# bayesml/BayesML

Measured on AMD Instinct MI355X. Metric: GMM-VB E+M samples/sec at K=64,D=128,N=1e7; 1/2/4/8-GPU scaling, higher is better.
Workload: dtype f64; 1 GPU; GMM-VB K=64 D=128 N=10000000 rows/GPU x 1 GPU, x stored f32, one VB iteration per step (c3 of BASELINE.json configs); classes=64, degree=128, rows_per_gpu=10000000, rows_total=10000000, x_storage=f32, parallelism=rows1, row_tiles=1

## Files before the change

### bayesml_amd/csrc/capi_estep.hip

```cpp
#include "capi_internal.h"

namespace {

struct Pass {
    gmmvb_workspace* ws;
    const void* x_dev;
    int64_t ldx, n_rows;
    hipStream_t st;
    int is64;
    bool vec;
    int sel_grid;
    double pairs;
    EstepArgs a{};
    EstepI8Args a8{};
    RecArrays rec{};
    bool i8 = false;
    bool prunable = false;
    bool prev_lists = false, can_project = false, own_known = false, tmeta_was_valid = false;
    bool quiet_was_valid = false;
    int mode = kPassDense;
    bool settle = false, proof_capable = false;
    double skip_margin = -1.0;
    bool counted = false, proof_ran = false, tmeta_kept = false, projected = false, filtered = false, emission_to_hmm = false,
         sorted_now = false;
// ... 116 lines not shown
                       estep_gather_rows_per_wg(ws->T, is64), ws->plan);
    hipError_t e = hipGetLastError();
    span_end(ws, st);
    if (e != hipSuccess) return e;
    span_begin(ws, kSpanGather, st);
    e = launch_estep_gather_dev(ws->T, is64, vec, 2 * ws->num_cu, st, a, ws->lists, ws->npad, ws->counts, ws->plan, thr,
                                thr ? ws->exit_ctr : nullptr, 0.0f);
    span_end(ws, st);
    ++ws->passes[7];
    return e;
}

}

extern "C" {


bool cal_wanted(gmmvb_workspace* ws, int what, double pairs) {
    return ws->opt_calibrate && ws->cal_ev[0] != nullptr && !((ws->pt.measured >> what) & 1) && ws->cal_pairs[what] == 0.0 &&
           pairs >= (double)(int64_t(1) << 23) && ws->hmm == nullptr;
}
void cal_mark(gmmvb_workspace* ws, int what, double pairs, hipStream_t st) {
    note_hip(ws, hipEventRecord(ws->cal_ev[2 * what + 1], st));
    ws->cal_pairs[what] = pairs;
}
void cal_poll(gmmvb_workspace* ws) {
    for (int what = 0; what < 3; ++what) {
        if (ws->cal_pairs[what] <= 0.0 || hipEventQuery(ws->cal_ev[2 * what + 1]) != hipSuccess) continue;
        float ms = 0.0f;
        if (hipEventElapsedTime(&ms, ws->cal_ev[2 * what], ws->cal_ev[2 * what + 1]) == hipSuccess) {
            double ns = (double)ms * 1e6 / ws->cal_pairs[what];
            if (what == 2) ns += 0.010 * tri_pairs(ws->T) / 36.0;
            const bool took = ws->pt.take(what, ns);
            if (ws->opt_debug)
                std::fprintf(stderr, "[gmmvb] policy table: %s %.4f ns per pair %s (prune below %.3f, dense again above %.3f, list M below %.3f)\n",
                             what == 0 ? "dense E" : (what == 1 ? "dense M" : "bound pass"), ns, took ? "taken" : "out of range: literal kept",
                             ws->pt.prune_below(), ws->pt.dense_again_above(), ws->pt.list_m_below());
            if (!took) ws->pt.measured |= 8 << what;
            ws->cal_pairs[what] = (took || ++ws->cal_tries[what] >= 3) ? -1.0 : 0.0;
        } else {
            ws->cal_pairs[what] = -1.0;
        }
    }
}

}

namespace {

hipError_t proof_round(gmmvb_workspace* ws, hipStream_t st, const int* blk_base, int sel_grid, int64_t n_rows, float* ub) {
    if (ws->opt_proof_blocked && ws->slabs &&
        estep_i8_proof_work_bytes(ws->K, n_rows) <= ws->scratch->bytes[kBuf_slabs])
        return launch_estep_i8_proof_blocked(ws->D, ws->num_cu, st, ws->xq, ws->xqe, ws->img_i8b, ws->cvec, ws->K, ws->lists,
                                             ws->npad, ws->counts, blk_base, sel_grid, ws->slabs, ub, ws->lnrho, ws->npad);
    hipLaunchKernelGGL(gather_plan_kernel, dim3(1), dim3(64), 0, st, ws->counts, ws->K, estep_i8_pairs_per_chunk(), ws->plan);
    return launch_estep_i8_proof(ws->D, ws->num_cu, st, ws->xq, ws->xqe, ws->img_i8b, ws->cvec, ws->K, ws->lists, ws->npad,
                                 ws->counts, ws->plan, ub, ws->lnrho, ws->npad);
}

int Pass::run_generic() {
    const int R = generic_rows(ws->D);
    const dim3 g((unsigned)((n_rows + R - 1) / R), (unsigned)ws->K);
    const size_t lds = (size_t)ws->D * R * sizeof(double);
    span_begin(ws, kSpanEstepMain, st);
    if (is64)
        hipLaunchKernelGGL(estep_generic_kernel<double>, g, dim3(64), lds, st, (const double*)x_dev, ldx, n_rows, ws->D,
                           ws->gen_u, ws->gen_m, ws->cvec, R, ws->lnrho, ws->npad);
    else
        hipLaunchKernelGGL(estep_generic_kernel<float>, g, dim3(64), lds, st, (const float*)x_dev, ldx, n_rows, ws->D,
                           ws->gen_u, ws->gen_m, ws->cvec, R, ws->lnrho, ws->npad);
    span_end(ws, st);
    if (phase_events(ws)) {
        note_hip(ws, hipEventRecord(ws->ev[1], st));
        ws->ev_e = true;
    }
    phase_closed = true;
    span_begin(ws, kSpanLse, st);
    hipLaunchKernelGGL(row_lse_kernel, dim3((unsigned)((n_rows + kLseRows - 1) / kLseRows)), dim3(256), 0, st, ws->lnrho,
                       ws->npad, n_rows, ws->K, ws->lse, nullptr, nullptr, 1);
    span_end(ws, st);
    hipError_t eg = hipGetLastError();
    if (eg != hipSuccess) return fail(GMMVB_EHIP, "estep_generic launch", eg);
    ++ws->passes[0];
    ws->rec_live = ws->rec_valid = false;
    ws->evaluated = pairs;
    std::snprintf(ws->info, sizeof(ws->info), "estep_generic_f64<D=%d> grid=%ux%ux64 rows/workgroup=%d", ws->D, g.x, g.y, R);
    name = nullptr;
    return GMMVB_OK;
}

int Pass::run_dense() {
    const bool valu16 = ws->estep_variant == kEstepValu16 && ws->tri != nullptr;
    emission_to_hmm = ws->T == 1 && !ws->wide && !i8 && !ws->sorted && hmm_fused_emission(ws->hmm);
    rpw = ws->wide ? estep_rows_rows_per_wg()
                     : (i8 ? estep_i8_rows_per_wg() : (valu16 ? estep_rows16_rows_per_wg() : estep_rows_per_wg(ws->estep_variant, ws->T, is64)));
    grid = (n_rows + rpw - 1) / rpw;
    if (grid > (1 << 20)) grid = 1 << 20;
    span_begin(ws, kSpanEstepMain, st);
    const bool cal_e = !ws->wide && !i8 && !emission_to_hmm && !valu16 && cal_wanted(ws, 0, pairs);
    if (cal_e) note_hip(ws, hipEventRecord(ws->cal_ev[0], st));
    hipError_t e = ws->wide ? launch_estep_rows(ws->T, is64, (int)grid, st, a, &name)
                            : (i8 ? launch_estep_i8(is64, vec, (int)grid, st, a8, &name)
                                  : (emission_to_hmm ? hmm_launch_emission16(ws->hmm, is64, vec, st, a, &name)
                                     : (valu16 ? launch_estep_rows16(is64, vec, (int)grid, st, a, ws->tri, &name)
                                            : launch_estep(ws->estep_variant, ws->T, is64, vec, (int)grid, st, a, &name))));
    if (cal_e) cal_mark(ws, 0, pairs, st);
    span_end(ws, st);
// ... 415 lines not shown
```

### bayesml_amd/csrc/estep_i8.h

```cpp
#pragma once
#include "common.h"

#include <type_traits>

namespace gmmvb {

typedef int i4v __attribute__((ext_vector_type(4)));
typedef int i16v __attribute__((ext_vector_type(16)));

constexpr int kDigits = 6;
constexpr int kBoundDigits = 3;

__host__ __device__ constexpr int i8_blocks(int D) { return (D + 31) / 32; }
__host__ __device__ constexpr int i8_img_bytes(int nd, int t32) {
    return (tri_pairs(t32) * nd * 1024 + (nd == kBoundDigits ? t32 * 128 + 32 : t32 * 512) + 1023) / 1024 * 1024;
}
__host__ __device__ constexpr int i8_kb(int nd, int t32) {
    const int kb = (64 * 1024) / i8_img_bytes(nd, t32);
    return kb < 1 ? 1 : (kb > 8 ? 8 : kb);
}
__host__ __device__ constexpr double i8_err(int nd, int t32) {
    double w = 1.0;
    for (int i = 0; i < 7 * nd; ++i) w *= 0.5;
    return w * (2.0 + 1.02 * (nd - 1)) * 32.0 * t32 * 1.000001;
}

template <int ND>
__device__ __forceinline__ void digits_of(double t, int (&d)[ND]) {
#pragma unroll
    for (int a = 0; a < ND; ++a) {
        const double r = __builtin_rint(t);
        d[a] = (int)r;
        t = (t - r) * 128.0;
    }
}

template <int ND>
__device__ __forceinline__ void pack_i8_image(const double* us, int ld, const double* dm, int D, int T32, int img_bytes,
                                              unsigned char* __restrict__ im, double* row_scale ,
                                              double* row_max, double* row_beta, int* row_bad) {
    const int P = tri_pairs(T32);
    double* consts = reinterpret_cast<double*>(im + P * ND * 1024);
    for (int j = threadIdx.x; j < 32 * T32; j += blockDim.x) {
        double mx = 0.0, bias = 0.0, abias = 0.0;
        bool bad = false;
        if (j < D) {
            for (int i = 0; i <= j; ++i) {
                const double v = us[j * ld + i];
                bad |= !(fabs(v) <= 1.7976931348623157e308);
                mx = fmax(mx, fabs(v));
                bias = fma(v, dm[i], bias);
                abias = fma(fabs(v), fabs(dm[i]), abias);
            }
        }
// ... 518 lines not shown
            const int64_t e = chunk0 + ((int64_t)t * NW + wave) * 32 + c;
            return list[e < count ? e : count - 1];
        };
        auto request = [&](int idx, i4v (&xd)[ND][T32], int64_t& row, int& en) {
            row = idx;
            const unsigned char* src = xq + row * RS + 16 * h;
#pragma unroll
            for (int a = 0; a < ND; ++a)
#pragma unroll
                for (int it = 0; it < T32; ++it) xd[a][it] = *reinterpret_cast<const i4v*>(src + a * 32 * T32 + 32 * it);
            en = xqe[row];
        };
        auto evaluate = [&](int t, const i4v (&xd)[ND][T32], int64_t row, int en) {
            const bool ok = en != kNoDigits;
            i8_lane_consts lc;
            lc.c[0] = lc.c[1] = lc.c[2] = 0.0;
            lc.c2f = ok ? (float)ldexp(1.0, en - 12 - 7 * (ND - 1)) : 0.0f;
            lc.cef = ok ? (float)(ldexp(1.0, en) * i8_err(ND, T32) * 1.0001) : __builtin_huge_valf();
            float q_lo, q_hi;
            if (T32 > 1 && wave >= NW / 2)
                estep_i8_two_sided<T32, true>(im_lds, xd, lc, lane, h, q_lo, q_hi);
            else
                estep_i8_two_sided<T32, false>(im_lds, xd, lc, lane, h, q_lo, q_hi);
            const int64_t e = chunk0 + ((int64_t)t * NW + wave) * 32 + c;
            if (h == 0 && e < count) {
                const double up = fma(-0.5 * (double)q_lo, 1.0 - 1.52587890625e-05, ck + 1e-12 * fabs(ck));
                const double lo = fma(-0.5 * (double)q_hi, 1.0 + 1.52587890625e-05, ck - 1e-12 * fabs(ck));
                if (ub) ub[(int64_t)k * npad + row] = __double2float_ru(up);
                lb[(int64_t)k * npad + row] = (lo == lo) ? lo : -__builtin_huge_val();
            }
        };
        i4v xa[ND][T32], xb[ND][T32];
        int64_t ra = 0, rb = 0;
        int ea = 0, eb = 0;
        int i1 = nt > 1 ? entry(1) : 0;
        if (nt > 0) request(entry(0), xa, ra, ea);
        for (int t = 0; t < nt; t += 2) {
            const int i2 = t + 2 < nt ? entry(t + 2) : 0;
            if (t + 1 < nt) request(i1, xb, rb, eb);
            evaluate(t, xa, ra, ea);
            if (t + 1 >= nt) break;
            const int i3 = t + 3 < nt ? entry(t + 3) : 0;
            if (t + 2 < nt) request(i2, xa, ra, ea);
            evaluate(t + 1, xb, rb, eb);
            i1 = i3;
        }
    }
}


constexpr int kProofSuperRows = 4096;
constexpr int kProofItem = 256;
constexpr int kProofXcds = 8;

__device__ __forceinline__ void proof_unit(const int* __restrict__ blk_base, const int* __restrict__ counts, int nblk, int s,
                                           int k, int K, int& lo, int& hi) {
    constexpr int BS = kProofSuperRows / 256;
    const int b0 = s * BS, b1 = b0 + BS;
    lo = blk_base[(int64_t)b0 * K + k];
    hi = b1 < nblk ? blk_base[(int64_t)b1 * K + k] : counts[k];
}

__global__ __launch_bounds__(256) void proof_units_kernel(const int* __restrict__ blk_base ,
                                                          const int* __restrict__ counts, int K, int nblk,
                                                          int* __restrict__ cum , int* __restrict__ tot) {
    __shared__ int sc[256];
    const int s = blockIdx.x, k = threadIdx.x;
    int n = 0;
    if (k < K) {
        int lo, hi;
        proof_unit(blk_base, counts, nblk, s, k, K, lo, hi);
        n = (hi - lo + kProofItem - 1) / kProofItem;
    }
    sc[k] = n;
    __syncthreads();
    for (int o = 1; o < 256; o <<= 1) {
        const int v = k >= o ? sc[k - o] : 0;
        __syncthreads();
        sc[k] += v;
        __syncthreads();
    }
    if (k < K) cum[(int64_t)s * (K + 1) + k] = sc[k] - n;
    if (k == 255) {
        cum[(int64_t)s * (K + 1) + K] = sc[255];
        tot[s] = sc[255];
    }
}

__global__ __launch_bounds__(1024) void proof_order_kernel(const int* __restrict__ tot, int n_super, int* __restrict__ xb,
                                                           int* __restrict__ xtot) {
    __shared__ int sc[1024];
    const int x = blockIdx.x, t = threadIdx.x;
    const int nx = n_super > x ? (n_super - x + kProofXcds - 1) / kProofXcds : 0;
    const int per = (nx + 1023) / 1024;
    const int j0 = t * per, j1 = j0 + per < nx ? j0 + per : nx;
    int sum = 0;
    for (int j = j0; j < j1; ++j) sum += tot[x + kProofXcds * j];
    sc[t] = sum;
    __syncthreads();
    for (int o = 1; o < 1024; o <<= 1) {
        const int v = t >= o ? sc[t - o] : 0;
        __syncthreads();
        sc[t] += v;
        __syncthreads();
    }
    int run = sc[t] - sum;
    for (int j = j0; j < j1; ++j) {
        xb[x + kProofXcds * j] = run;
        run += tot[x + kProofXcds * j];
    }
    if (t == 1023) xtot[x] = sc[1023];
}

__global__ __launch_bounds__(256) void proof_items_kernel(const int* __restrict__ blk_base, const int* __restrict__ counts, int K,
                                                          int nblk, const int* __restrict__ cum, const int* __restrict__ xb,
                                                          const int* __restrict__ xtot, i4v* __restrict__ items) {
    const int s = blockIdx.x, k = threadIdx.x;
    if (k >= K) return;
    int first = 0;
    for (int q = 0; q < s % kProofXcds; ++q) first += xtot[q];
    int lo, hi;
    proof_unit(blk_base, counts, nblk, s, k, K, lo, hi);
    i4v* dst = items + first + xb[s] + cum[(int64_t)s * (K + 1) + k];
    for (int e = lo; e < hi; e += kProofItem) *dst++ = i4v{k, e, hi - e < kProofItem ? hi - e : kProofItem, s};
}

template <int T32>
__global__ __launch_bounds__(512) void estep_i8_proof_blocked(const unsigned char* __restrict__ xq, const signed char* __restrict__ xqe,
                                                              const unsigned char* __restrict__ img ,
                                                              const double* __restrict__ cvec, int K,
                                                              const int* __restrict__ lists , int64_t cap,
                                                              const i4v* __restrict__ items, const int* __restrict__ xtot,
                                                              float* __restrict__ ub , double* __restrict__ lb ,
                                                              int64_t npad) {
    constexpr int ND = kBoundDigits, NW = 8;
    constexpr int IMGB = i8_img_bytes(ND, T32);
    constexpr int64_t RS = i8_digit_row_bytes(T32);
    constexpr int NS = T32 <= 3 ? 3 : 2;
    constexpr int NI = (IMGB + 512 * 16 - 1) / (512 * 16);
    __shared__ __attribute__((aligned(16))) unsigned char smem[2][IMGB];
    const int tid = threadIdx.x;
    const int lane = tid & 63;
    const int wave = __builtin_amdgcn_readfirstlane(tid >> 6);
    const int c = lane & 31, h = lane >> 5;
    const int x = (int)(blockIdx.x % kProofXcds), j = (int)(blockIdx.x / kProofXcds), W = (int)(gridDim.x / kProofXcds);
    int first = 0;
    for (int q = 0; q < x; ++q) first += xtot[q];
    const int n_items = xtot[x];
    const i4v* my = items + first;
    if (n_items <= j) return;
    auto desc = [&](int t) -> i4v {
        const int i = j + t * W;
        i4v d = my[i < n_items ? i : n_items - 1];
        if (i >= n_items) d[3] = -1;
        return d;
    };
    auto entry = [&](const i4v& d) -> int {
        const int o = wave * 32 + c;
        return lists[(int64_t)d[0] * cap + d[1] + (o < d[2] ? o : d[2] - 1)];
    };
    auto image_load = [&](int k, i4v (&ir)[NI]) {
        const unsigned char* src = img + (int64_t)k * IMGB;
#pragma unroll
        for (int q = 0; q < NI; ++q) {
            const int o = (q * 512 + tid) * 16;
            ir[q] = *reinterpret_cast<const i4v*>(src + (o < IMGB ? o : IMGB - 16));
        }
    };
    auto image_store = [&](int buf, const i4v (&ir)[NI]) {
#pragma unroll
        for (int q = 0; q < NI; ++q)
            if ((q * 512 + tid) * 16 < IMGB) *reinterpret_cast<i4v*>(&smem[buf][(q * 512 + tid) * 16]) = ir[q];
    };
    auto request = [&](int idx, i4v (&xd)[ND][T32], int64_t& row, int& en) {
        row = idx;
        const unsigned char* src = xq + row * RS + 16 * h;
#pragma unroll
        for (int a = 0; a < ND; ++a)
#pragma unroll
            for (int it = 0; it < T32; ++it) xd[a][it] = *reinterpret_cast<const i4v*>(src + a * 32 * T32 + 32 * it);
        en = xqe[row];
    };
    auto evaluate = [&](const i4v& d, int buf, const i4v (&xd)[ND][T32], int64_t row, int en) {
        if (d[3] < 0 || wave * 32 >= d[2]) return;
        const unsigned im_lds = (unsigned)(uintptr_t)((__attribute__((address_space(3))) unsigned char*)smem[buf]);
        const bool ok = en != kNoDigits;
        i8_lane_consts lc;
        lc.c[0] = lc.c[1] = lc.c[2] = 0.0;
        lc.c2f = ok ? (float)ldexp(1.0, en - 12 - 7 * (ND - 1)) : 0.0f;
        lc.cef = ok ? (float)(ldexp(1.0, en) * i8_err(ND, T32) * 1.0001) : __builtin_huge_valf();
        float q_lo, q_hi;
        if (T32 > 1 && wave >= NW / 2)
            estep_i8_two_sided<T32, true>(im_lds, xd, lc, lane, h, q_lo, q_hi);
        else
            estep_i8_two_sided<T32, false>(im_lds, xd, lc, lane, h, q_lo, q_hi);
        if (h == 0 && wave * 32 + c < d[2]) {
            const int k = d[0];
            const double ck = cvec[k];
            const double up = fma(-0.5 * (double)q_lo, 1.0 - 1.52587890625e-05, ck + 1e-12 * fabs(ck));
            const double lo = fma(-0.5 * (double)q_hi, 1.0 + 1.52587890625e-05, ck - 1e-12 * fabs(ck));
            if (ub) ub[(int64_t)k * npad + row] = __double2float_ru(up);
            lb[(int64_t)k * npad + row] = (lo == lo) ? lo : -__builtin_huge_val();
        }
    };
    i4v xs[NS][ND][T32];
    int64_t rows[NS];
    int ens[NS];
    i4v dd[NS + 2];
#pragma unroll
    for (int i = 0; i < NS + 2; ++i) dd[i] = desc(i);
    i4v ir[NI];
    image_load(dd[0][0], ir);
#pragma unroll
    for (int q = 0; q < NS; ++q) {
        rows[q] = 0;
        ens[q] = 0;
        if (q + 1 < NS) request(entry(dd[q]), xs[q], rows[q], ens[q]);
    }
    int e_next = entry(dd[NS - 1]);
    constexpr int UNR = (T32 <= 2 ? 4 : 2) * NS;
    for (int t = 0; dd[0][3] >= 0; t += UNR) {
#pragma unroll
        for (int p = 0; p < UNR; ++p) {
            const int buf = (t + p) & 1;
            image_store(buf, ir);
            __syncthreads();
            image_load(dd[1][0], ir);
            const int e_new = entry(dd[NS]);
            request(e_next, xs[(p + NS - 1) % NS], rows[(p + NS - 1) % NS], ens[(p + NS - 1) % NS]);
            e_next = e_new;
            const i4v dn = desc(t + p + NS + 2);
            evaluate(dd[0], buf, xs[p % NS], rows[p % NS], ens[p % NS]);
#pragma unroll
            for (int i = 0; i < NS + 1; ++i) dd[i] = dd[i + 1];
            dd[NS + 1] = dn;
        }
    }
}

}
```

### bayesml_amd/csrc/estep_i8_inst.hip

```cpp
#include <cstdint>
#include <cstdlib>
#include <mutex>
#include "aux_kernels.h"
#include "estep_i8.h"
#include "launch.h"

namespace gmmvb {

int estep_i8_image_bytes(int D, int bound) { return i8_img_bytes(bound ? kBoundDigits : kDigits, i8_blocks(D)); }
int estep_i8_rows_per_wg() { return 8 * 32; }

constexpr int kPackThreads = 512;
__global__ __launch_bounds__(kPackThreads) void pack_images_kernel(const double* __restrict__ u, const double* __restrict__ m,
                                                                    const double* __restrict__ c_src, const double* __restrict__ pivot_src,
                                                                    int K, int D, int T, int img_len, double* __restrict__ img,
                                                                    double* __restrict__ c_dst, double* __restrict__ pivot_dst,
                                                                    int T32, unsigned char* __restrict__ img6, int img6_bytes,
                                                                    unsigned char* __restrict__ img3, int img3_bytes) {
    extern __shared__ double us[];
    __shared__ double row_scale[128], row_max[128], row_beta[128];
    __shared__ int row_bad[128];
    const int k = blockIdx.x, kind = blockIdx.y;
    const int ld = D | 1;
    double* mv = us + D * ld;
    const double* uk = u + (int64_t)k * D * D;
    for (int e = threadIdx.x; e < D * D; e += kPackThreads) {
        const int i = e / D, j = e - i * D;
        if (j <= i) us[i * ld + j] = uk[e];
    }
    for (int i = threadIdx.x; i < D; i += kPackThreads) {
        const double mi = m[(int64_t)k * D + i];
        mv[i] = kind == 0 ? mi : mi - pivot_src[i];
    }
    __syncthreads();
    if (kind == 0) {
        if (threadIdx.x == 0) c_dst[k] = c_src[k];
        if (pivot_dst && k == 0)
            for (int f = threadIdx.x; f < D; f += kPackThreads) pivot_dst[f] = pivot_src[f];
        pack_f64_image(us, ld, mv, D, T, img_len, img + (int64_t)k * img_len);
    } else if (kind == 1 && img6) {
        pack_i8_image<kDigits>(us, ld, mv, D, T32, img6_bytes, img6 + (int64_t)k * img6_bytes, row_scale, row_max, row_beta, row_bad);
    } else {
        pack_i8_image<kBoundDigits>(us, ld, mv, D, T32, img3_bytes, img3 + (int64_t)k * img3_bytes, row_scale, row_max, row_beta,
                                    row_bad);
    }
}

hipError_t launch_pack_images(const double* u, const double* m, const double* c_src, const double* pivot_src, int K, int D, int T,
                              int img_len, double* img, double* cvec, double* pivot_dst, unsigned char* img6, unsigned char* img3,
                              hipStream_t st) {
    if (D > 128 || ((img6 || img3) && !pivot_dst)) return hipErrorInvalidValue;
    static std::mutex mu;
    static bool asked[64] = {};
    int dev = 0;
    hipError_t e = hipGetDevice(&dev);
    if (e != hipSuccess) return e;
    {
        std::lock_guard<std::mutex> lock(mu);
// ... 51 lines not shown
    if (t32 < 1 || t32 > 4 || tb < 1 || tb > t32) return hipErrorInvalidValue;
    *name = names[t32][tb];
#define BC(T, B) \
    if (t32 == T && tb == B) return pick_x<kBoundDigits, true, T, B>(x_is_f64, vec, grid, st, a);
    BC(1, 1) BC(2, 1) BC(2, 2) BC(3, 1) BC(3, 2) BC(3, 3) BC(4, 1) BC(4, 2) BC(4, 3) BC(4, 4)
#undef BC
    return hipErrorInvalidValue;
}

int64_t estep_i8_digit_row_bytes(int D) { return i8_digit_row_bytes(i8_blocks(D)); }

hipError_t launch_x_digits(const void* x, int x_is_f64, int64_t ldx, int64_t n_rows, int D, const double* pivot,
                           unsigned char* xq, signed char* xqe, hipStream_t st) {
    const int t32 = i8_blocks(D);
    if (t32 < 1 || t32 > 4) return hipErrorInvalidValue;
    const unsigned grid = (unsigned)((n_rows + 31) / 32);
    if (x_is_f64)
        hipLaunchKernelGGL(x_digits_kernel<double>, dim3(grid), dim3(256), 0, st, static_cast<const double*>(x), ldx, n_rows, D,
                           t32, pivot, xq, xqe);
    else
        hipLaunchKernelGGL(x_digits_kernel<float>, dim3(grid), dim3(256), 0, st, static_cast<const float*>(x), ldx, n_rows, D,
                           t32, pivot, xq, xqe);
    return hipGetLastError();
}

int estep_i8_pairs_per_chunk() { return i8_pairs_per_chunk(); }

hipError_t launch_estep_i8_proof(int D, int grid, hipStream_t st, const unsigned char* xq, const signed char* xqe,
                                 const unsigned char* img, const double* cvec, int K, const int* lists, int64_t cap,
                                 const int* counts, const int* plan, float* ub, double* lb, int64_t npad) {
    if (K > 256) return hipErrorInvalidValue;
    grid *= 2;
#define PC(T)                                                                                                              \
    case T:                                                                                                                \
        hipLaunchKernelGGL((estep_i8_proof<T>), dim3(grid), dim3(512), 0, st, xq, xqe, img, cvec, K, lists, cap, counts,   \
                           plan, ub, lb, npad);                                                                            \
        return hipGetLastError();
    switch (i8_blocks(D)) {
        PC(1) PC(2) PC(3) PC(4)
    }
#undef PC
    return hipErrorInvalidValue;
}


int64_t estep_i8_proof_work_bytes(int K, int64_t n_rows) {
    const int64_t nblk = (n_rows + 255) / 256;
    const int64_t n_super = (nblk * 256 + kProofSuperRows - 1) / kProofSuperRows;
    const int64_t head = ((2 * n_super + kProofXcds + 3) / 4 * 4 + (n_super * (K + 1) + 3) / 4 * 4) * (int64_t)sizeof(int);
    const int64_t items = n_rows * (int64_t)K / kProofItem + n_super * K + 1;
    return head + items * (int64_t)sizeof(i4v);
}

hipError_t launch_estep_i8_proof_blocked(int D, int num_cu, hipStream_t st, const unsigned char* xq, const signed char* xqe,
                                         const unsigned char* img, const double* cvec, int K, const int* lists, int64_t cap,
                                         const int* counts, const int* blk_base, int nblk, void* work, float* ub, double* lb,
                                         int64_t npad) {
    if (K > 256 || nblk < 1 || !work || ((uintptr_t)work & 15)) return hipErrorInvalidValue;
    const int n_super = (int)(((int64_t)nblk * 256 + kProofSuperRows - 1) / kProofSuperRows);
    int* tot = static_cast<int*>(work);
    int* xb = tot + n_super;
    int* xtot = xb + n_super;
    int* cum = tot + (2 * (int64_t)n_super + kProofXcds + 3) / 4 * 4;
    i4v* items = reinterpret_cast<i4v*>(cum + ((int64_t)n_super * (K + 1) + 3) / 4 * 4);
    hipLaunchKernelGGL(proof_units_kernel, dim3(n_super), dim3(256), 0, st, blk_base, counts, K, nblk, cum, tot);
    hipLaunchKernelGGL(proof_order_kernel, dim3(kProofXcds), dim3(1024), 0, st, tot, n_super, xb, xtot);
    hipLaunchKernelGGL(proof_items_kernel, dim3(n_super), dim3(256), 0, st, blk_base, counts, K, nblk, cum, xb, xtot, items);
    const int per_cu = i8_blocks(D) == 1 ? 2 : 1;
    const int grid = kProofXcds * ((per_cu * num_cu + kProofXcds - 1) / kProofXcds);
#define PB(T)                                                                                                              \
    case T:                                                                                                                \
        hipLaunchKernelGGL((estep_i8_proof_blocked<T>), dim3(grid), dim3(512), 0, st, xq, xqe, img, cvec, K, lists, cap,   \
                           items, xtot, ub, lb, npad);                                                                     \
        return hipGetLastError();
    switch (i8_blocks(D)) {
        PB(1) PB(2) PB(3) PB(4)
    }
#undef PB
    return hipErrorInvalidValue;
}

}
```

### bayesml_amd/csrc/launch.h

```cpp
#pragma once
#include <hip/hip_runtime.h>
#include <stdint.h>

#include "workspace_plan.h"

struct gmmvb_hmm_state;

namespace gmmvb {

struct EstepArgs {
    const void* x; int64_t ldx; int64_t n_rows; int D;
    const double* img; const double* cvec; int K;
    double* lnrho; int64_t npad;
};
struct MstepArgs {
    const void* x; int64_t ldx; int64_t n_rows; int D;
    const double* pivot; const double* lnrho; const double* lse; const double* aux; int64_t npad;
    int K; int KG; int S; int64_t rows_per_split; int direct_r; double* slabs;
};

int estep_rows_per_wg(int variant, int T, int x_is_f64);
int estep_threads(int variant);
int estep_image_doubles(int T);
int estep_tri_image_doubles();
int estep_rows16_rows_per_wg();
hipError_t launch_pack_tri16(const double* u, const double* m, int K, int D, double* tri, hipStream_t st);
hipError_t launch_estep_rows16(int x_is_f64, bool vec, int grid, hipStream_t st, const EstepArgs& a, const double* tri,
                               const char** name);
hipError_t hmm_launch_emission16(::gmmvb_hmm_state* h, int x_is_f64, bool vec, hipStream_t st, const EstepArgs& a, const char** name);
int estep_bound_blocks(int T);
int estep_gather_rows_per_wg(int T, int x_is_f64);
hipError_t launch_estep_gather_dev(int T, int x_is_f64, bool vec, int grid, hipStream_t st, const EstepArgs& a,
                                   const int* lists, int64_t cap, const int* counts_dev, const int* plan_dev,
                                   const float* thr = nullptr ,
                                   unsigned long long* exits = nullptr ,
                                   float margin = 0.0f );
int64_t estep_i8_digit_row_bytes(int D);
hipError_t launch_x_digits(const void* x, int x_is_f64, int64_t ldx, int64_t n_rows, int D, const double* pivot,
                           unsigned char* xq, signed char* xqe, hipStream_t st);
int64_t proj_image_len(int K, int D);
int64_t proj_const_len(int K);
hipError_t launch_proj_table(const double* u, const double* m, const double* cvec, const double* pivot, int K, int D,
                             unsigned char* gimg, void* gconst, hipStream_t st);
hipError_t launch_proj_tile_ref(const int* counts, int K, int64_t n_tiles, int* tile_ref, hipStream_t st);
struct ProjectArgs {
    const unsigned char* xq; const signed char* xqe;
    const unsigned char* gimg; const void* gconst; const int* tile_ref;
    const double* lnrho; int64_t npad; int64_t n_rows; int K; int D; const double* drift; const double* cvec;
    unsigned short* rec_k; float* rec_d; float* rec_B; unsigned char* rec_exact; unsigned char* rec_sel; unsigned char* rec_flags;
    unsigned long long* masks; int* blk; double* epart; double* opart;
    unsigned char* lock; float* dlock; float* rthr; const unsigned char* lcomp;
    unsigned long long* pmask; int* pblk; int proof_all; int own_fresh; unsigned long long* cand_ctr;
};
hipError_t launch_rec_project(int grid, hipStream_t st, const ProjectArgs& a);
hipError_t launch_proj_filter(int grid, hipStream_t st, const ProjectArgs& a);
int estep_i8_pairs_per_chunk();
hipError_t launch_estep_i8_proof(int D, int grid, hipStream_t st, const unsigned char* xq, const signed char* xqe,
                                 const unsigned char* img, const double* cvec, int K, const int* lists, int64_t cap,
                                 const int* counts, const int* plan, float* ub, double* lb, int64_t npad);
int64_t estep_i8_proof_work_bytes(int K, int64_t n_rows);
hipError_t launch_estep_i8_proof_blocked(int D, int num_cu, hipStream_t st, const unsigned char* xq, const signed char* xqe,
                                         const unsigned char* img, const double* cvec, int K, const int* lists, int64_t cap,
                                         const int* counts, const int* blk_base, int nblk, void* work, float* ub, double* lb,
                                         int64_t npad);
struct EstepI8Args {
    const void* x; int64_t ldx; int64_t n_rows; int D;
    const unsigned char* img; const double* pivot; const double* cvec; int K;
    double* lnrho; int64_t npad;
    int* khat = nullptr;
    float* ub = nullptr;
};
int estep_i8_image_bytes(int D, int bound);
int estep_i8_rows_per_wg();
hipError_t launch_pack_images(const double* u, const double* m, const double* c_src, const double* pivot_src, int K, int D, int T,
                              int img_len, double* img, double* cvec, double* pivot_dst, unsigned char* img6, unsigned char* img3,
                              hipStream_t st);
hipError_t launch_estep_i8(int x_is_f64, bool vec, int grid, hipStream_t st, const EstepI8Args& a, const char** name);
hipError_t launch_estep_i8_bound(int x_is_f64, bool vec, int tb, int grid, hipStream_t st, const EstepI8Args& a,
                                 const char** name);
int mstep_components_per_wg(int T, bool pre);
int mstep_threads(int T, bool pre);
hipError_t launch_estep(int variant, int T, int x_is_f64, bool vec, int grid, hipStream_t st, const EstepArgs& a,
                        const char** name);
hipError_t launch_mstep(int T, int x_is_f64, bool vec, bool pre, int grid, hipStream_t st, const MstepArgs& a,
                        const char** name);

hipError_t launch_mstep_small(int grid, hipStream_t st, const MstepArgs& a, int KGW, int cw, const char** name);
hipError_t launch_mstep_wide(int T, int grid, hipStream_t st, const MstepArgs& a, const char** name);
hipError_t launch_estep_rows(int T, int x_is_f64, int grid, hipStream_t st, const EstepArgs& a, const char** name);
int estep_rows_rows_per_wg();
hipError_t launch_hmm_mstep_small(int grid, hipStream_t st, const MstepArgs& a, int KGW, const double* gamma_tm, int Kp,
                                  bool sparse, const char** name);

struct MstepListArgs {
    const double* xc; const double* lnrho; const double* lse;
    const int* lists; int64_t cap; const int* counts; int* plan; int cap_chunks; int r_min;
    int64_t npad; int K; double* slabs;
    const float* x32 = nullptr; int64_t ldx = 0; int64_t n_rows = 0; int D = 0; const double* pivot = nullptr;
    int direct_r = 0;
    int num_cu = 0;
    int runs_cap = 0;
};
hipError_t launch_mstep_list(int T, int grid, hipStream_t st, const MstepListArgs& a, const char** name, int* runs);

}
```

### bayesml_amd/csrc/workspace_plan.h

```cpp
#pragma once
#include <stdint.h>

#include <algorithm>
#include <cstdlib>
#include <cstring>
#include <type_traits>
#include <vector>

#include "../../include/gmmvb.h"

namespace gmmvb {

enum EstepVariant { kEstepLds = 0, kEstepDirect = 1, kEstepLds8 = 2, kEstepI8 = 3, kEstepValu16 = 4 };
inline int64_t round_up(int64_t v, int64_t m) { return (v + m - 1) / m * m; }

inline bool not_zero(const char* v) { return !(v && std::strcmp(v, "0") == 0); }
inline bool is(const char* v, const char* word) { return v && std::strcmp(v, word) == 0; }
template <typename Lookup>
inline const char* dev_switch(Lookup&& lookup, const char* name) {
    const char* on = lookup("GMMVB_DEBUG");
    return (on && on[0] != '\0' && on[0] != '0') ? lookup(name) : nullptr;
}

struct WorkspaceOptions {
    bool sparse = true;
    int prune = 1;
    int variant_asked = -1;
    bool sort_rows = true;
    double settle_margin = 1e300;
    bool opt_proof = true;
    bool opt_proof_all = true;
    bool opt_proof_blocked = true;
    bool opt_lazy = true;
    int opt_project = 0;
    bool opt_regroup_margin = true;
    bool gather_exit = true;
    bool cache_on = true;
    bool opt_carry_off = false;
    bool opt_hmm_mstep_dense = false;
    bool opt_calibrate = true;
    bool opt_quiet_tiles = true;
    bool opt_mlist_xc = false;
    int opt_mlist_runs = 0;
    int opt_sweep_run = 0;
    bool opt_debug = false;

    template <typename Lookup>
    static WorkspaceOptions read(Lookup&& lookup) {
        auto dev = [&lookup](const char* name) { return dev_switch(lookup, name); };
        WorkspaceOptions o;
        o.sparse = not_zero(lookup("GMMVB_MSTEP_SPARSE"));
        o.prune = is(lookup("GMMVB_ESTEP_PRUNE"), "0") ? 0 : (is(lookup("GMMVB_ESTEP_PRUNE"), "force") ? 2 : 1);
        const char* variant = dev("GMMVB_ESTEP_VARIANT");
        o.variant_asked = is(variant, "lds8") ? kEstepLds8 : is(variant, "direct") ? kEstepDirect : is(variant, "lds4") ? kEstepLds
                          : is(variant, "i8") ? kEstepI8 : -1;
        o.sort_rows = not_zero(dev("GMMVB_SORT_ROWS"));
        if (const char* v = dev("GMMVB_SETTLE_MARGIN")) o.settle_margin = std::atof(v);
        o.opt_proof = not_zero(dev("GMMVB_PROOF"));
        o.opt_proof_all = !is(dev("GMMVB_PROOF"), "settled");
        o.opt_proof_blocked = not_zero(dev("GMMVB_PROOF_BLOCKED"));
        o.opt_lazy = not_zero(dev("GMMVB_SWEEP_LAZY"));
        o.opt_project = is(dev("GMMVB_PROJECT"), "filter") ? 1 : (is(dev("GMMVB_PROJECT"), "only") ? 2 : 0);
        o.opt_regroup_margin = not_zero(dev("GMMVB_REGROUP_MARGIN"));
        o.gather_exit = not_zero(dev("GMMVB_GATHER_EXIT"));
        o.cache_on = not_zero(dev("GMMVB_MSTEP_CACHE"));
        o.opt_carry_off = dev("GMMVB_ESTEP_CARRY_OFF") != nullptr;
        o.opt_hmm_mstep_dense = dev("GMMVB_HMM_MSTEP_DENSE") != nullptr;
        o.opt_calibrate = not_zero(dev("GMMVB_POLICY_CALIBRATE"));
        o.opt_quiet_tiles = not_zero(dev("GMMVB_QUIET_TILES"));
        if (const char* v = dev("GMMVB_MLIST_XC")) o.opt_mlist_xc = v[0] == '1';
        if (const char* v = dev("GMMVB_MLIST_RUNS")) o.opt_mlist_runs = std::max(0, std::atoi(v));
        if (const char* v = dev("GMMVB_SWEEP_RUN")) o.opt_sweep_run = std::max(0, std::atoi(v));
        o.opt_debug = lookup("GMMVB_DEBUG") && lookup("GMMVB_DEBUG")[0] == '2';
        return o;
    }
};

constexpr int kSweepRunDefault = 2;
inline int sweep_run_length(int K, int asked) {
    if (K > 128) return 1;
    const int want = asked > 0 ? asked : kSweepRunDefault;
    return want >= 4 ? 4 : (want >= 2 ? 2 : 1);
}
template <typename F>
inline void dispatch_sweep_run(int run, F&& f) {
    if (run == 4) return f(std::integral_constant<int, 4>{});
    if (run == 2) return f(std::integral_constant<int, 2>{});
    return f(std::integral_constant<int, 1>{});
}

struct KernelSizes {
    int max_tiles = 0, t1_splits = 0, sel_rows = 0, lse_rows = 0, scan_parts = 0, rec_slots = 0;
    int mstep_components_per_wg = 0;
    int slab_len = 0, estep_image_doubles = 0, estep_tri_image_doubles = 0, estep_bound_blocks = 0;
    int estep_i8_image_bytes = 0, estep_i8_bound_image_bytes = 0;
    int64_t estep_i8_digit_row_bytes = 0, proj_image_len = 0, proj_const_len = 0;
    int generic_rows = 0;
};

inline bool wide_features(int D, int max_tiles) { return D > 16 * max_tiles && D <= 32 * max_tiles; }
inline int feature_tiles(int D, int max_tiles) {
    const int T = (D + 15) / 16;
    return wide_features(D, max_tiles) ? 2 * ((T + 1) / 2) : T;
}

struct WorkspaceShape : WorkspaceOptions {
    int K = 0, D = 0, x_dtype = 0, num_cu = 0, T = 0;
    int64_t max_rows = 0, npad = 0;
    bool wide = false;
    bool generic = false;
    int KG = 0, S_cap = 0, img_len = 0, estep_variant = 0, gen_S = 1, img_i8_len = 0, img_i8b_len = 0;
    int64_t split_rows = 0, xc_len = 0;
    bool has_lists = false;
};

inline WorkspaceShape make_shape(int K, int D, int x_dtype, int64_t max_rows, int num_cu, const WorkspaceOptions& opt,
                                 const KernelSizes& ks) {
    WorkspaceShape s;
    s.K = K;
    s.D = D;
    s.x_dtype = x_dtype;
    s.max_rows = max_rows;
    s.num_cu = num_cu;
    s.T = feature_tiles(D, ks.max_tiles);
    s.wide = wide_features(D, ks.max_tiles);
    s.generic = D > 32 * ks.max_tiles;
    s.npad = round_up(max_rows, 64);
    if (s.generic) {
        s.sparse = s.sort_rows = s.cache_on = false;
        s.prune = 0;
        s.gen_S = (int)std::min<int64_t>(64, std::max<int64_t>(1, max_rows / 16384));
        return s;
    }
    static_cast<WorkspaceOptions&>(s) = opt;
    s.KG = (K + ks.mstep_components_per_wg - 1) / ks.mstep_components_per_wg;
    s.S_cap = std::max(8, (int)round_up(((int64_t)(s.T == 1 ? ks.t1_splits : 4) * num_cu + s.KG - 1) / s.KG, 8));
    s.split_rows = round_up(std::max<int64_t>(64, (16 << 20) / (16 * s.T * 8)), 64);
    s.S_cap = (int)std::max<int64_t>(s.S_cap, round_up((max_rows + s.split_rows - 1) / s.split_rows, 8));
    s.img_len = ks.estep_image_doubles;
    s.estep_variant = s.T == 1 ? kEstepValu16 : kEstepLds8;
    if (!s.wide && opt.variant_asked >= 0) s.estep_variant = opt.variant_asked;
// ... 195 lines not shown
```

Measured before the change: 6.580 billion samples/s.

## Assign contiguous item stretches per workgroup in blocked proof and skip redundant image restaging

```diff
diff --git a/bayesml_amd/csrc/capi_estep.hip b/bayesml_amd/csrc/capi_estep.hip
--- a/bayesml_amd/csrc/capi_estep.hip
+++ b/bayesml_amd/csrc/capi_estep.hip
@@ -192,7 +192,8 @@
     if (ws->opt_proof_blocked && ws->slabs &&
         estep_i8_proof_work_bytes(ws->K, n_rows) <= ws->scratch->bytes[kBuf_slabs])
         return launch_estep_i8_proof_blocked(ws->D, ws->num_cu, st, ws->xq, ws->xqe, ws->img_i8b, ws->cvec, ws->K, ws->lists,
-                                             ws->npad, ws->counts, blk_base, sel_grid, ws->slabs, ub, ws->lnrho, ws->npad);
+                                             ws->npad, ws->counts, blk_base, sel_grid, ws->slabs, ws->opt_proof_run, ws->opt_debug,
+                                             ub, ws->lnrho, ws->npad);
     hipLaunchKernelGGL(gather_plan_kernel, dim3(1), dim3(64), 0, st, ws->counts, ws->K, estep_i8_pairs_per_chunk(), ws->plan);
     return launch_estep_i8_proof(ws->D, ws->num_cu, st, ws->xq, ws->xqe, ws->img_i8b, ws->cvec, ws->K, ws->lists, ws->npad,
                                  ws->counts, ws->plan, ub, ws->lnrho, ws->npad);
diff --git a/bayesml_amd/csrc/estep_i8.h b/bayesml_amd/csrc/estep_i8.h
--- a/bayesml_amd/csrc/estep_i8.h
+++ b/bayesml_amd/csrc/estep_i8.h
@@ -1,5 +1,6 @@
 #pragma once
 #include "common.h"
+#include "workspace_plan.h"
 
 #include <type_traits>
 
@@ -624,6 +625,7 @@
 constexpr int kProofSuperRows = 4096;
 constexpr int kProofItem = 256;
 constexpr int kProofXcds = 8;
+static_assert(kProofRunMax == kProofSuperRows / kProofItem, "a stretch holds at most the items of one full unit");
 
 __device__ __forceinline__ void proof_unit(const int* __restrict__ blk_base, const int* __restrict__ counts, int nblk, int s,
                                            int k, int K, int& lo, int& hi) {
@@ -703,6 +705,7 @@
                                                               const double* __restrict__ cvec, int K,
                                                               const int* __restrict__ lists , int64_t cap,
                                                               const i4v* __restrict__ items, const int* __restrict__ xtot,
+                                                              int run_asked ,
                                                               float* __restrict__ ub , double* __restrict__ lb ,
                                                               int64_t npad) {
     constexpr int ND = kBoundDigits, NW = 8;
@@ -720,9 +723,15 @@
     for (int q = 0; q < x; ++q) first += xtot[q];
     const int n_items = xtot[x];
     const i4v* my = items + first;
-    if (n_items <= j) return;
-    auto desc = [&](int t) -> i4v {
-        const int i = j + t * W;
+    const int G = proof_run_length(n_items, W, run_asked);
+    if (n_items <= j * G) return;
+    int nx_base = j * G, nx_off = 0;
+    auto next_desc = [&]() -> i4v {
+        const int i = nx_base + nx_off;
+        if (++nx_off == G) {
+            nx_off = 0;
+            nx_base += W * G;
+        }
         i4v d = my[i < n_items ? i : n_items - 1];
         if (i >= n_items) d[3] = -1;
         return d;
@@ -780,7 +789,7 @@
     int ens[NS];
     i4v dd[NS + 2];
 #pragma unroll
-    for (int i = 0; i < NS + 2; ++i) dd[i] = desc(i);
+    for (int i = 0; i < NS + 2; ++i) dd[i] = next_desc();
     i4v ir[NI];
     image_load(dd[0][0], ir);
 #pragma unroll
@@ -791,17 +800,21 @@
     }
     int e_next = entry(dd[NS - 1]);
     constexpr int UNR = (T32 <= 2 ? 4 : 2) * NS;
-    for (int t = 0; dd[0][3] >= 0; t += UNR) {
+    int staged = -1, buf = 1;
+    while (dd[0][3] >= 0) {
 #pragma unroll
         for (int p = 0; p < UNR; ++p) {
-            const int buf = (t + p) & 1;
-            image_store(buf, ir);
-            __syncthreads();
+            if (dd[0][0] != staged) {
+                buf ^= 1;
+                image_store(buf, ir);
+                __syncthreads();
+                staged = dd[0][0];
+            }
             image_load(dd[1][0], ir);
             const int e_new = entry(dd[NS]);
             request(e_next, xs[(p + NS - 1) % NS], rows[(p + NS - 1) % NS], ens[(p + NS - 1) % NS]);
             e_next = e_new;
-            const i4v dn = desc(t + p + NS + 2);
+            const i4v dn = next_desc();
             evaluate(dd[0], buf, xs[p % NS], rows[p % NS], ens[p % NS]);
 #pragma unroll
             for (int i = 0; i < NS + 1; ++i) dd[i] = dd[i + 1];
diff --git a/bayesml_amd/csrc/estep_i8_inst.hip b/bayesml_amd/csrc/estep_i8_inst.hip
--- a/bayesml_amd/csrc/estep_i8_inst.hip
+++ b/bayesml_amd/csrc/estep_i8_inst.hip
@@ -1,4 +1,5 @@
 #include <cstdint>
+#include <cstdio>
 #include <cstdlib>
 #include <mutex>
 #include "aux_kernels.h"
@@ -161,10 +162,47 @@
     return head + items * (int64_t)sizeof(i4v);
 }
 
+static void proof_units_report(hipStream_t st, const int* xtot, const i4v* items, int grid, int run_asked) {
+    int xt[kProofXcds];
+    if (hipStreamSynchronize(st) != hipSuccess || hipMemcpy(xt, xtot, sizeof(xt), hipMemcpyDeviceToHost) != hipSuccess) return;
+    int64_t n = 0;
+    int most = 0;
+    for (int v : xt) {
+        n += v;
+        most = std::max(most, v);
+    }
+    std::vector<i4v> it((size_t)n);
+    if (n > 0 && hipMemcpy(it.data(), items, (size_t)n * sizeof(i4v), hipMemcpyDeviceToHost) != hipSuccess) return;
+    constexpr int EB = 9;
+    const int edge[EB] = {8, 16, 32, 64, 128, 256, 1024, 2048, 4096};
+    int64_t by_entries[EB] = {}, by_items[kProofRunMax + 1] = {}, units = 0, in_long_units = 0, pairs = 0;
+    for (int64_t i = 0; i < n;) {
+        int64_t e = i;
+        int entries = 0;
+        while (e < n && it[e][0] == it[i][0] && it[e][3] == it[i][3]) entries += it[e++][2];
+        const int ni = (int)(e - i);
+        ++units;
+        pairs += entries;
+        if (ni >= 2) in_long_units += ni;
+        ++by_items[ni < kProofRunMax ? ni : kProofRunMax];
+        int b = 0;
+        while (b + 1 < EB && entries > edge[b]) ++b;
+        ++by_entries[b];
+        i = e;
+    }
+    std::fprintf(stderr, "[gmmvb] proof units: pairs %lld units %lld items %lld in_units_of_2_or_more %lld G %d | entries<=8,16,32,64,128,256,1024,2048,4096:",
+                 (long long)pairs, (long long)units, (long long)n, (long long)in_long_units,
+                 proof_run_length(most, std::max(1, grid / kProofXcds), run_asked));
+    for (int b = 0; b < EB; ++b) std::fprintf(stderr, " %lld", (long long)by_entries[b]);
+    std::fprintf(stderr, " | items per unit 1..%d:", kProofRunMax);
+    for (int b = 1; b <= kProofRunMax; ++b) std::fprintf(stderr, " %lld", (long long)by_items[b]);
+    std::fprintf(stderr, "\n");
+}
+
 hipError_t launch_estep_i8_proof_blocked(int D, int num_cu, hipStream_t st, const unsigned char* xq, const signed char* xqe,
                                          const unsigned char* img, const double* cvec, int K, const int* lists, int64_t cap,
-                                         const int* counts, const int* blk_base, int nblk, void* work, float* ub, double* lb,
-                                         int64_t npad) {
+                                         const int* counts, const int* blk_base, int nblk, void* work, int run_asked, bool report,
+                                         float* ub, double* lb, int64_t npad) {
     if (K > 256 || nblk < 1 || !work || ((uintptr_t)work & 15)) return hipErrorInvalidValue;
     const int n_super = (int)(((int64_t)nblk * 256 + kProofSuperRows - 1) / kProofSuperRows);
     int* tot = static_cast<int*>(work);
@@ -180,13 +218,16 @@
 #define PB(T)                                                                                                              \
     case T:                                                                                                                \
         hipLaunchKernelGGL((estep_i8_proof_blocked<T>), dim3(grid), dim3(512), 0, st, xq, xqe, img, cvec, K, lists, cap,   \
-                           items, xtot, ub, lb, npad);                                                                     \
-        return hipGetLastError();
+                           items, xtot, run_asked, ub, lb, npad);                                                            \
+        break;
     switch (i8_blocks(D)) {
         PB(1) PB(2) PB(3) PB(4)
+        default: return hipErrorInvalidValue;
     }
 #undef PB
-    return hipErrorInvalidValue;
-}
-
-}
+    const hipError_t e = hipGetLastError();
+    if (report && e == hipSuccess) proof_units_report(st, xtot, items, grid, run_asked);
+    return e;
+}
+
+}
diff --git a/bayesml_amd/csrc/launch.h b/bayesml_amd/csrc/launch.h
--- a/bayesml_amd/csrc/launch.h
+++ b/bayesml_amd/csrc/launch.h
@@ -61,8 +61,8 @@
 int64_t estep_i8_proof_work_bytes(int K, int64_t n_rows);
 hipError_t launch_estep_i8_proof_blocked(int D, int num_cu, hipStream_t st, const unsigned char* xq, const signed char* xqe,
                                          const unsigned char* img, const double* cvec, int K, const int* lists, int64_t cap,
-                                         const int* counts, const int* blk_base, int nblk, void* work, float* ub, double* lb,
-                                         int64_t npad);
+                                         const int* counts, const int* blk_base, int nblk, void* work, int run_asked, bool report,
+                                         float* ub, double* lb, int64_t npad);
 struct EstepI8Args {
     const void* x; int64_t ldx; int64_t n_rows; int D;
     const unsigned char* img; const double* pivot; const double* cvec; int K;
diff --git a/bayesml_amd/csrc/workspace_plan.h b/bayesml_amd/csrc/workspace_plan.h
--- a/bayesml_amd/csrc/workspace_plan.h
+++ b/bayesml_amd/csrc/workspace_plan.h
@@ -43,6 +43,7 @@
     bool opt_mlist_xc = false;
     int opt_mlist_runs = 0;
     int opt_sweep_run = 0;
+    int opt_proof_run = 0;
     bool opt_debug = false;
 
     template <typename Lookup>
@@ -71,6 +72,7 @@
         if (const char* v = dev("GMMVB_MLIST_XC")) o.opt_mlist_xc = v[0] == '1';
         if (const char* v = dev("GMMVB_MLIST_RUNS")) o.opt_mlist_runs = std::max(0, std::atoi(v));
         if (const char* v = dev("GMMVB_SWEEP_RUN")) o.opt_sweep_run = std::max(0, std::atoi(v));
+        if (const char* v = dev("GMMVB_PROOF_RUN")) o.opt_proof_run = std::max(0, std::atoi(v));
         o.opt_debug = lookup("GMMVB_DEBUG") && lookup("GMMVB_DEBUG")[0] == '2';
         return o;
     }
@@ -87,6 +89,14 @@
     if (run == 4) return f(std::integral_constant<int, 4>{});
     if (run == 2) return f(std::integral_constant<int, 2>{});
     return f(std::integral_constant<int, 1>{});
+}
+
+constexpr int kProofRunMax = 16;
+constexpr int kProofRunsPerWorkgroup = 16;
+constexpr int proof_run_length(int n_items, int W, int asked) {
+    int g = asked > 0 ? asked : ((n_items > 0 && W > 0) ? n_items / W / kProofRunsPerWorkgroup : 1);
+    if (g > kProofRunMax) g = kProofRunMax;
+    return g < 1 ? 1 : g;
 }
 
 struct KernelSizes {
```

Result: no change. 6.627 billion samples/s, median of 2 (+0.7%).

## Group consecutive proof items per block and skip redundant component image reloads

Applied to the files above, without the earlier changes.

```diff
diff --git a/bayesml_amd/csrc/capi_estep.hip b/bayesml_amd/csrc/capi_estep.hip
--- a/bayesml_amd/csrc/capi_estep.hip
+++ b/bayesml_amd/csrc/capi_estep.hip
@@ -192,7 +192,8 @@
     if (ws->opt_proof_blocked && ws->slabs &&
         estep_i8_proof_work_bytes(ws->K, n_rows) <= ws->scratch->bytes[kBuf_slabs])
         return launch_estep_i8_proof_blocked(ws->D, ws->num_cu, st, ws->xq, ws->xqe, ws->img_i8b, ws->cvec, ws->K, ws->lists,
-                                             ws->npad, ws->counts, blk_base, sel_grid, ws->slabs, ub, ws->lnrho, ws->npad);
+                                             ws->npad, ws->counts, blk_base, sel_grid, ws->slabs, ub, ws->lnrho, ws->npad,
+                                             proof_group_length((ws->D + 31) / 32, ws->opt_proof_group));
     hipLaunchKernelGGL(gather_plan_kernel, dim3(1), dim3(64), 0, st, ws->counts, ws->K, estep_i8_pairs_per_chunk(), ws->plan);
     return launch_estep_i8_proof(ws->D, ws->num_cu, st, ws->xq, ws->xqe, ws->img_i8b, ws->cvec, ws->K, ws->lists, ws->npad,
                                  ws->counts, ws->plan, ub, ws->lnrho, ws->npad);
diff --git a/bayesml_amd/csrc/estep_i8.h b/bayesml_amd/csrc/estep_i8.h
--- a/bayesml_amd/csrc/estep_i8.h
+++ b/bayesml_amd/csrc/estep_i8.h
@@ -697,7 +697,7 @@
     for (int e = lo; e < hi; e += kProofItem) *dst++ = i4v{k, e, hi - e < kProofItem ? hi - e : kProofItem, s};
 }
 
-template <int T32>
+template <int T32, int G>
 __global__ __launch_bounds__(512) void estep_i8_proof_blocked(const unsigned char* __restrict__ xq, const signed char* __restrict__ xqe,
                                                               const unsigned char* __restrict__ img ,
                                                               const double* __restrict__ cvec, int K,
@@ -720,9 +720,9 @@
     for (int q = 0; q < x; ++q) first += xtot[q];
     const int n_items = xtot[x];
     const i4v* my = items + first;
-    if (n_items <= j) return;
+    if (n_items <= j * G) return;
     auto desc = [&](int t) -> i4v {
-        const int i = j + t * W;
+        const int i = (j + (t / G) * W) * G + t % G;
         i4v d = my[i < n_items ? i : n_items - 1];
         if (i >= n_items) d[3] = -1;
         return d;
@@ -731,7 +731,8 @@
         const int o = wave * 32 + c;
         return lists[(int64_t)d[0] * cap + d[1] + (o < d[2] ? o : d[2] - 1)];
     };
-    auto image_load = [&](int k, i4v (&ir)[NI]) {
+    auto image_load = [&](int k, bool whole, i4v (&ir)[NI]) {
+        if (!whole) return;
         const unsigned char* src = img + (int64_t)k * IMGB;
 #pragma unroll
         for (int q = 0; q < NI; ++q) {
@@ -782,7 +783,7 @@
 #pragma unroll
     for (int i = 0; i < NS + 2; ++i) dd[i] = desc(i);
     i4v ir[NI];
-    image_load(dd[0][0], ir);
+    image_load(dd[0][0], true, ir);
 #pragma unroll
     for (int q = 0; q < NS; ++q) {
         rows[q] = 0;
@@ -791,13 +792,19 @@
     }
     int e_next = entry(dd[NS - 1]);
     constexpr int UNR = (T32 <= 2 ? 4 : 2) * NS;
+    int buf = 1;
+    bool starts = true;
     for (int t = 0; dd[0][3] >= 0; t += UNR) {
 #pragma unroll
         for (int p = 0; p < UNR; ++p) {
-            const int buf = (t + p) & 1;
-            image_store(buf, ir);
-            __syncthreads();
-            image_load(dd[1][0], ir);
+            if (starts) {
+                buf ^= 1;
+                image_store(buf, ir);
+                __syncthreads();
+            }
+            starts = __builtin_amdgcn_readfirstlane(dd[1][3]) >= 0 &&
+                     __builtin_amdgcn_readfirstlane(dd[1][0]) != __builtin_amdgcn_readfirstlane(dd[0][0]);
+            image_load(dd[1][0], starts, ir);
             const int e_new = entry(dd[NS]);
             request(e_next, xs[(p + NS - 1) % NS], rows[(p + NS - 1) % NS], ens[(p + NS - 1) % NS]);
             e_next = e_new;
diff --git a/bayesml_amd/csrc/estep_i8_inst.hip b/bayesml_amd/csrc/estep_i8_inst.hip
--- a/bayesml_amd/csrc/estep_i8_inst.hip
+++ b/bayesml_amd/csrc/estep_i8_inst.hip
@@ -4,6 +4,7 @@
 #include "aux_kernels.h"
 #include "estep_i8.h"
 #include "launch.h"
+#include "workspace_plan.h"
 
 namespace gmmvb {
 
@@ -164,7 +165,7 @@
 hipError_t launch_estep_i8_proof_blocked(int D, int num_cu, hipStream_t st, const unsigned char* xq, const signed char* xqe,
                                          const unsigned char* img, const double* cvec, int K, const int* lists, int64_t cap,
                                          const int* counts, const int* blk_base, int nblk, void* work, float* ub, double* lb,
-                                         int64_t npad) {
+                                         int64_t npad, int group) {
     if (K > 256 || nblk < 1 || !work || ((uintptr_t)work & 15)) return hipErrorInvalidValue;
     const int n_super = (int)(((int64_t)nblk * 256 + kProofSuperRows - 1) / kProofSuperRows);
     int* tot = static_cast<int*>(work);
@@ -179,8 +180,10 @@
     const int grid = kProofXcds * ((per_cu * num_cu + kProofXcds - 1) / kProofXcds);
 #define PB(T)                                                                                                              \
     case T:                                                                                                                \
-        hipLaunchKernelGGL((estep_i8_proof_blocked<T>), dim3(grid), dim3(512), 0, st, xq, xqe, img, cvec, K, lists, cap,   \
-                           items, xtot, ub, lb, npad);                                                                     \
+        dispatch_proof_group(group, [&](auto gg) {                                                                         \
+            hipLaunchKernelGGL((estep_i8_proof_blocked<T, decltype(gg)::value>), dim3(grid), dim3(512), 0, st, xq, xqe,    \
+                               img, cvec, K, lists, cap, items, xtot, ub, lb, npad);                                       \
+        });                                                                                                                \
         return hipGetLastError();
     switch (i8_blocks(D)) {
         PB(1) PB(2) PB(3) PB(4)
diff --git a/bayesml_amd/csrc/launch.h b/bayesml_amd/csrc/launch.h
--- a/bayesml_amd/csrc/launch.h
+++ b/bayesml_amd/csrc/launch.h
@@ -62,7 +62,7 @@
 hipError_t launch_estep_i8_proof_blocked(int D, int num_cu, hipStream_t st, const unsigned char* xq, const signed char* xqe,
                                          const unsigned char* img, const double* cvec, int K, const int* lists, int64_t cap,
                                          const int* counts, const int* blk_base, int nblk, void* work, float* ub, double* lb,
-                                         int64_t npad);
+                                         int64_t npad, int group);
 struct EstepI8Args {
     const void* x; int64_t ldx; int64_t n_rows; int D;
     const unsigned char* img; const double* pivot; const double* cvec; int K;
diff --git a/bayesml_amd/csrc/workspace_plan.h b/bayesml_amd/csrc/workspace_plan.h
--- a/bayesml_amd/csrc/workspace_plan.h
+++ b/bayesml_amd/csrc/workspace_plan.h
@@ -43,6 +43,7 @@
     bool opt_mlist_xc = false;
     int opt_mlist_runs = 0;
     int opt_sweep_run = 0;
+    int opt_proof_group = 0;
     bool opt_debug = false;
 
     template <typename Lookup>
@@ -71,6 +72,7 @@
         if (const char* v = dev("GMMVB_MLIST_XC")) o.opt_mlist_xc = v[0] == '1';
         if (const char* v = dev("GMMVB_MLIST_RUNS")) o.opt_mlist_runs = std::max(0, std::atoi(v));
         if (const char* v = dev("GMMVB_SWEEP_RUN")) o.opt_sweep_run = std::max(0, std::atoi(v));
+        if (const char* v = dev("GMMVB_PROOF_GROUP")) o.opt_proof_group = std::max(0, std::atoi(v));
         o.opt_debug = lookup("GMMVB_DEBUG") && lookup("GMMVB_DEBUG")[0] == '2';
         return o;
     }
@@ -86,6 +88,19 @@
 inline void dispatch_sweep_run(int run, F&& f) {
     if (run == 4) return f(std::integral_constant<int, 4>{});
     if (run == 2) return f(std::integral_constant<int, 2>{});
+    return f(std::integral_constant<int, 1>{});
+}
+
+inline int proof_group_default(int t32) { return t32 >= 2 ? 4 : 1; }
+inline int proof_group_length(int t32, int asked) {
+    const int want = asked > 0 ? asked : proof_group_default(t32);
+    return want >= 8 ? 8 : (want >= 4 ? 4 : (want >= 2 ? 2 : 1));
+}
+template <typename F>
+inline void dispatch_proof_group(int group, F&& f) {
+    if (group == 8) return f(std::integral_constant<int, 8>{});
+    if (group == 4) return f(std::integral_constant<int, 4>{});
+    if (group == 2) return f(std::integral_constant<int, 2>{});
     return f(std::integral_constant<int, 1>{});
 }
 
```

New measurement: 6.605 billion samples/s before, 6.595 billion samples/s after. No clear change (-0.1%).
